# arcosoph/nanowakeword

Hardware: AMD Instinct MI355X
Metric: clips/sec (1 s @16 kHz PCM->logits) (higher is better)
Workload: dtype f32; 1 GPU; cnn head on (101,64) log-mel, batch=4096/GPU, 1 s 16 kHz mono int16 clips, 64-mel 25 ms/10 ms center frontend, fused STFT+mel HIP kernel, fp32; clips_per_gpu=4096, n_samples=16000, parallelism=batch-split x1

## Files before the change

### nanowakeword_amd/csrc/fe_steps.h

```cpp
#pragma once
#include <math.h>
#include <stdint.h>

#if defined(__HIPCC__)
#include <hip/hip_runtime.h>
#define NWW_HD __host__ __device__ __forceinline__
typedef float2 nww_c32;
#else
#define NWW_HD inline
struct nww_c32 { float x, y; };
#endif

#define FE_NFFT 400
#define FE_M 200
#define FE_BINS 201
#define FE_PSTRIDE 209
#define FE_MAX_MELS 128
#define FE_MAX_MELW 640

NWW_HD nww_c32 c_make(float x, float y) { nww_c32 r; r.x = x; r.y = y; return r; }
NWW_HD nww_c32 c_add(nww_c32 a, nww_c32 b) { return c_make(a.x + b.x, a.y + b.y); }
NWW_HD nww_c32 c_sub(nww_c32 a, nww_c32 b) { return c_make(a.x - b.x, a.y - b.y); }
NWW_HD nww_c32 c_mul(nww_c32 a, nww_c32 b) { return c_make(a.x * b.x - a.y * b.y, a.x * b.y + a.y * b.x); }
NWW_HD nww_c32 c_mul_negi(nww_c32 a) { return c_make(a.y, -a.x); }
NWW_HD nww_c32 c_scale(nww_c32 a, float s) { return c_make(a.x * s, a.y * s); }

struct FeTables {
    nww_c32 win2[FE_M];
    nww_c32 tw200[8 * 25];
    nww_c32 tw400[101];
    int32_t mel_lo[FE_MAX_MELS];
    int32_t mel_cnt[FE_MAX_MELS];
    int32_t mel_off[FE_MAX_MELS];
    float melw[FE_MAX_MELW];
};

NWW_HD void dft8(nww_c32 z[8]) {
    const float r = 0.70710678118654752440f;
    nww_c32 a0 = c_add(z[0], z[4]), a1 = c_add(z[1], z[5]), a2 = c_add(z[2], z[6]), a3 = c_add(z[3], z[7]);
    nww_c32 b0 = c_sub(z[0], z[4]);
    nww_c32 d1 = c_sub(z[1], z[5]), d2 = c_sub(z[2], z[6]), d3 = c_sub(z[3], z[7]);
    nww_c32 b1 = c_make((d1.x + d1.y) * r, (d1.y - d1.x) * r);
    nww_c32 b2 = c_mul_negi(d2);
    nww_c32 b3 = c_make((d3.y - d3.x) * r, -(d3.x + d3.y) * r);
    nww_c32 p0 = c_add(a0, a2), p1 = c_sub(a0, a2), q0 = c_add(a1, a3), q1 = c_mul_negi(c_sub(a1, a3));
    z[0] = c_add(p0, q0); z[4] = c_sub(p0, q0); z[2] = c_add(p1, q1); z[6] = c_sub(p1, q1);
    nww_c32 s0 = c_add(b0, b2), s1 = c_sub(b0, b2), t0 = c_add(b1, b3), t1 = c_mul_negi(c_sub(b1, b3));
    z[1] = c_add(s0, t0); z[5] = c_sub(s0, t0); z[3] = c_add(s1, t1); z[7] = c_sub(s1, t1);
}

NWW_HD void dft5(nww_c32& x0, nww_c32& x1, nww_c32& x2, nww_c32& x3, nww_c32& x4) {
    const float c1 = 0.30901699437494742410f, c2 = -0.80901699437494742410f;
    const float s1 = 0.95105651629515357212f, s2 = 0.58778525229247312917f;
    nww_c32 a1 = c_add(x1, x4), a2 = c_add(x2, x3), b1 = c_sub(x1, x4), b2 = c_sub(x2, x3);
    nww_c32 m1 = c_make(x0.x + c1 * a1.x + c2 * a2.x, x0.y + c1 * a1.y + c2 * a2.y);
    nww_c32 m2 = c_make(x0.x + c2 * a1.x + c1 * a2.x, x0.y + c2 * a1.y + c1 * a2.y);
    nww_c32 n1 = c_make(s1 * b1.x + s2 * b2.x, s1 * b1.y + s2 * b2.y);
    nww_c32 n2 = c_make(s2 * b1.x - s1 * b2.x, s2 * b1.y - s1 * b2.y);
    nww_c32 j1 = c_mul_negi(n1), j2 = c_mul_negi(n2);
    x0 = c_make(x0.x + a1.x + a2.x, x0.y + a1.y + a2.y);
    x1 = c_add(m1, j1); x4 = c_sub(m1, j1);
    x2 = c_add(m2, j2); x3 = c_sub(m2, j2);
}

NWW_HD nww_c32 w25(int p) {
    const float C[17] = {1.0f, 0.96858316112863108f, 0.87630668004386358f, 0.72896862742141155f,
                         0.53582679497899666f, 0.30901699437494742f, 0.06279051952931337f,
                         -0.18738131458572463f, -0.42577929156507272f, -0.63742398974868975f,
                         -0.80901699437494742f, -0.92977648588825146f, -0.99211470131447788f,
                         -0.99211470131447788f, -0.92977648588825146f, -0.80901699437494742f,
                         -0.63742398974868975f};
    const float S[17] = {0.0f, 0.24868988716485479f, 0.48175367410171532f, 0.68454710592868873f,
                         0.84432792550201508f, 0.95105651629515357f, 0.99802672842827156f,
                         0.98228725072868872f, 0.90482705246601958f, 0.77051324277578925f,
                         0.58778525229247313f, 0.36812455268467797f, 0.12533323356430426f,
                         -0.12533323356430426f, -0.36812455268467797f, -0.58778525229247313f,
                         -0.77051324277578925f};
    return c_make(C[p], -S[p]);
}

#if defined(__HIP_DEVICE_COMPILE__)
#define NWW_SCHED_FENCE() __builtin_amdgcn_sched_barrier(0)
#else
#define NWW_SCHED_FENCE() ((void)0)
#endif
template <bool SEQ = false, typename LoadF, typename StoreF>
NWW_HD void dft25(LoadF load, StoreF store) {
    nww_c32 u[5][5];
#pragma unroll
    for (int b = 0; b < 5; ++b)
#pragma unroll
        for (int a = 0; a < 5; ++a) u[b][a] = load(5 * a + b);
#pragma unroll
    for (int b = 0; b < 5; ++b) {
        if (SEQ) NWW_SCHED_FENCE();
        dft5(u[b][0], u[b][1], u[b][2], u[b][3], u[b][4]);
        if (b > 0) {
#pragma unroll
            for (int c = 1; c < 5; ++c) u[b][c] = c_mul(u[b][c], w25(b * c));
        }
    }
#pragma unroll
    for (int c = 0; c < 5; ++c) {
        if (SEQ) NWW_SCHED_FENCE();
        dft5(u[0][c], u[1][c], u[2][c], u[3][c], u[4][c]);
#pragma unroll
        for (int d = 0; d < 5; ++d) store(c + 5 * d, u[d][c]);
    }
    if (SEQ) NWW_SCHED_FENCE();
}

NWW_HD void fe_s1(int f, int n2, int hop, const int16_t* span, const FeTables* tb, nww_c32* yz) {
    const uint32_t* fr = (const uint32_t*)(span + hop * f);
    nww_c32 z[8];
#pragma unroll
    for (int n1 = 0; n1 < 8; ++n1) {
        const int m = 25 * n1 + n2;
        const nww_c32 w = tb->win2[m];
        const uint32_t v = fr[m];
        z[n1] = c_make((float)(int16_t)(v & 0xffffu) * w.x, (float)(int16_t)(v >> 16) * w.y);
    }
    dft8(z);
    nww_c32* out = yz + (f * 8) * 25 + n2;
    out[0] = z[0];
#pragma unroll
    for (int k1 = 1; k1 < 8; ++k1) out[k1 * 25] = c_mul(z[k1], tb->tw200[k1 * 25 + n2]);
}

NWW_HD void fe_s2(int f, int k1, nww_c32* yz) {
    nww_c32* row = yz + (f * 8 + k1) * 25;
    dft25([&](int i) { return row[i]; }, [&](int i, nww_c32 v) { row[i] = v; });
}

NWW_HD void fe_s3_core(nww_c32 A, nww_c32 B, nww_c32 tw, float* pa, float* pb) {
    const nww_c32 E = c_make(A.x + B.x, A.y - B.y);
    const nww_c32 O = c_make(A.y + B.y, B.x - A.x);
    const nww_c32 wO = c_mul(tw, O);
    const nww_c32 Xa = c_add(E, wO), Xb = c_sub(E, wO);
    *pa = Xa.x * Xa.x + Xa.y * Xa.y;
    *pb = Xb.x * Xb.x + Xb.y * Xb.y;
}
NWW_HD int fe_zpos(int k) { return (k & 7) * 25 + (k >> 3); }

NWW_HD void fe_s3(int f, int k, const FeTables* tb, const nww_c32* yz, float* pw) {
    const nww_c32* zf = yz + f * 200;
    const int kb = (k == 0) ? 0 : 200 - k;
    float* p = pw + f * FE_PSTRIDE;
    fe_s3_core(zf[fe_zpos(k)], zf[fe_zpos(kb)], tb->tw400[k], &p[k], &p[200 - k]);
}

NWW_HD float fe_s4(int f, int j, const FeTables* tb, const float* pw) {
    const float* p = pw + f * FE_PSTRIDE + tb->mel_lo[j];
    const float* w = tb->melw + tb->mel_off[j];
    const int n = tb->mel_cnt[j];
    float acc = 0.0f;
    for (int i = 0; i < n; ++i) acc = fmaf(p[i], w[i], acc);
    return acc;
}

NWW_HD float fe_db(float mel, float amin, float mult) {
    return mult * log10f(fmaxf(mel, amin));
}

NWW_HD int fe_reflect(int s, int N) {
    if (s < 0) s = -s;
    if (s >= N) s = 2 * (N - 1) - s;
    return s;
}

#define FE2_G 8
#define FE2_FRAME_DW 400
#define FE2_PSHIFT(f) (4 * ((f) >> 1))
#define FE2_STAGE_OFF 216
#define FE2_MAX_TILES 8
#define FE2_MAX_STEPS 512

#define FE2_CHUNK 8
#define FE2_MAX_CHUNKS 64
struct Fe2MelPlan {
    int32_t ntiles;
    int32_t total_steps;
    int32_t nchunks;
    int32_t tile_k0[FE2_MAX_TILES];
    int32_t tile_nsteps[FE2_MAX_TILES];
    int32_t tile_first[FE2_MAX_TILES];
    uint32_t chunk_meta[FE2_MAX_CHUNKS];
    float b[FE2_MAX_STEPS * 64];
};

NWW_HD void fe2_s1(const uint32_t s[8], const nww_c32 win[8], const nww_c32 tw[7], nww_c32 z[8]) {
#pragma unroll
    for (int n1 = 0; n1 < 8; ++n1)
        z[n1] = c_make((float)(int16_t)(s[n1] & 0xffffu) * win[n1].x, (float)(int16_t)(s[n1] >> 16) * win[n1].y);
    dft8(z);
#pragma unroll
    for (int k1 = 1; k1 < 8; ++k1) z[k1] = c_mul(z[k1], tw[k1 - 1]);
}

NWW_HD float fe2_mel_planned(const Fe2MelPlan* pl, const float* p, int j) {
    const int t = j >> 4, n = j & 15;
    const int k0 = pl->tile_k0[t], ns = pl->tile_nsteps[t];
    const float* b = pl->b + (size_t)pl->tile_first[t] * 64 + n;
    float acc[2] = {0.0f, 0.0f};
    for (int s = 0; s < ns; ++s)
        for (int kk = 0; kk < 4; ++kk) acc[s & 1] = fmaf(p[k0 + 4 * s + kk], b[s * 64 + kk * 16], acc[s & 1]);
    return acc[0] + acc[1];
}
```

### nanowakeword_amd/csrc/frontend2.hip

```cpp
#include <hip/hip_runtime.h>
#include <stdlib.h>
#include "fe_steps.h"
#include "frontend.h"
#include "layers.h"

typedef float f32x4 __attribute__((ext_vector_type(4)));

struct Fe2MelLds {
    uint32_t desc[FE_MAX_MELS];
    float w[FE_MAX_MELW];
};

__device__ __forceinline__ void fe2_wave_sync() {
    __builtin_amdgcn_fence(__ATOMIC_RELEASE, "wavefront");
    __builtin_amdgcn_wave_barrier();
    __builtin_amdgcn_fence(__ATOMIC_ACQUIRE, "wavefront");
}

__device__ __forceinline__ void fe2_load_column(const int16_t* __restrict__ x, int base, int n2, uint32_t v[8]) {
    const uint32_t* p = reinterpret_cast<const uint32_t*>(x + base) + n2;
#pragma unroll
    for (int n1 = 0; n1 < 8; ++n1) v[n1] = p[25 * n1];
}

__device__ __forceinline__ float fe2_db(float mel, float amin, float mult, float floor_db) {
    const float db = (mult * 0.30102999566398120f) * __log2f(fmaxf(mel, amin));
    return mel > amin ? db : floor_db;
}

#define FE2_PARAMS                                                                                                      \
    const int16_t *__restrict__ pcm, size_t row_stride, int B, int N, int T, int ngroups, int hop, int pad, int n_mels,    \
        float amin, float db_mult, float floor_db, const FeTables *__restrict__ gtb, const Fe2MelPlan *__restrict__ plan,  \
        float *__restrict__ out_db, float *__restrict__ out_mel, int frames_major, int dbg, int gsz, Fe2Sub sub
#define FE2_ARGS pcm, row_stride, B, N, T, ngroups, hop, pad, n_mels, amin, db_mult, floor_db, gtb, plan, out_db, out_mel, frames_major, dbg, gsz, sub
template <int MEL, int FAST_OUT, int MAXT, bool RING, bool FLAT>
__device__ __forceinline__ void fe2_wave_body(FE2_PARAMS) {
    static_assert(!FLAT || (FAST_OUT && !RING && MEL == 2), "flat items: frames-major fast output, register filters, no frame subsets");
#ifndef NWW_ABLATION
    if (FLAT) dbg = 0;
#endif
    extern __shared__ __attribute__((aligned(16))) char smem[];
    constexpr int MFMA_MEL = MEL == 1;
    const int lane = threadIdx.x & 63;
    const int wv = __builtin_amdgcn_readfirstlane((int)(threadIdx.x >> 6));
    const int nwv = blockDim.x >> 6;
    const int tb_bytes = MEL == 0 ? (int)sizeof(Fe2MelLds) : 0;
    Fe2MelLds* mt = reinterpret_cast<Fe2MelLds*>(smem);
    float* slab = reinterpret_cast<float*>(smem + tb_bytes) + wv * (FE2_G * FE2_FRAME_DW);
    if (MEL == 0) {
        for (int i = threadIdx.x; i < FE_MAX_MELS; i += blockDim.x)
            mt->desc[i] = (uint32_t)gtb->mel_lo[i] | ((uint32_t)gtb->mel_cnt[i] << 8) | ((uint32_t)gtb->mel_off[i] << 16);
        for (int i = threadIdx.x; i < FE_MAX_MELW; i += blockDim.x) mt->w[i] = gtb->melw[i];
        __syncthreads();
    }
    const int n2 = lane % 25, slot = lane / 25;
    nww_c32 win[8], tw[7];
#pragma unroll
    for (int n1 = 0; n1 < 8; ++n1) win[n1] = gtb->win2[25 * n1 + n2];
#pragma unroll
    for (int k1 = 1; k1 < 8; ++k1) tw[k1 - 1] = gtb->tw200[k1 * 25 + n2];
    const int k3a = lane, k3b = 64 + lane;
    const bool has_b = k3b <= 100;
    const nww_c32 twa = gtb->tw400[k3a], twb = gtb->tw400[has_b ? k3b : 100];
    const int ia2 = k3a ? FE_M - k3a : 0;
    const int f2 = lane >> 3, k1_2 = lane & 7;
    constexpr int NCO = FLAT ? 2 : 4;
    int co_off[NCO];
#pragma unroll
    for (int r = 0; r < NCO; ++r) {
        const int i = 4 * lane + 256 * r, f = i / n_mels, j = i - f * n_mels;
        co_off[r] = f * FE2_FRAME_DW + FE2_STAGE_OFF + FE2_PSHIFT(f) + j;
    }
    const int mel_l5 = lane & 31;
    const int mel_j = (lane & 32) + ((mel_l5 < 4) ? mel_l5 : (mel_l5 < 12) ? 12 + mel_l5 : (mel_l5 < 16) ? mel_l5 - 8 : (mel_l5 < 20) ? 8 + mel_l5
                                     : (mel_l5 < 28) ? mel_l5 - 12 : mel_l5);
    float wreg[MAXT];
    int mel_lo_lane = 0;
    if (MEL == 2) {
        const int j = min(mel_j, n_mels - 1);
        const int lo = gtb->mel_lo[j], sh4 = lo & 3;
        mel_lo_lane = lo - sh4;
        const int cnt = mel_j < n_mels ? gtb->mel_cnt[j] : 0, off = gtb->mel_off[j];
#pragma unroll
        for (int i = 0; i < MAXT; ++i) wreg[i] = (i >= sh4 && i - sh4 < cnt) ? gtb->melw[off + i - sh4] : 0.0f;
    }
    const int mel_nchunks = MFMA_MEL ? plan->nchunks : 0;
    const uint32_t mel_meta = MFMA_MEL ? plan->chunk_meta[lane] : 0u;
    const bool aligned = ((reinterpret_cast<uintptr_t>(pcm) | (row_stride * sizeof(int16_t))) & 3) == 0;

    const int total = FLAT ? (B * T + FE2_G - 1) / FE2_G : B * ngroups;
    const int stride = gridDim.x * nwv;
    uint32_t cur[8];
    auto geom = [&](int item, int& b, int& t0, int& nf) {
        b = item / ngroups;
        const int g = item - b * ngroups;
        if (!RING || sub.nr == 0) {
            t0 = g * gsz;
            nf = min(gsz, T - t0);
        } else {
            int r = 0;
            while (r + 1 < sub.nr && g >= sub.gend[r]) ++r;
            t0 = sub.t0[r] + (g - (r ? sub.gend[r - 1] : 0)) * gsz;
            nf = min(gsz, sub.t1[r] - t0);
        }
    };
    auto interior = [&](int t0, int nf) {
        const int s0 = t0 * hop - pad;
        return aligned && s0 >= 0 && s0 + (nf - 1) * hop + FE_NFFT <= N;
    };
    auto prefetch_first = [&](int item) {
        int b, t0, nf;
        geom(item, b, t0, nf);
        if (interior(t0, nf) && slot < nf && slot < 2)
            fe2_load_column(pcm + (size_t)b * row_stride, (t0 + slot) * hop - pad, n2, cur);
    };
    auto flat_frame = [&](int t0, int nf, int k, uint32_t& woff, int& s0) {
        int f = 2 * k + slot;
        if (nf < FE2_G) f = min(f, nf - 1);
        int t = t0 + f;
        woff = 0u;
        if (t0 + FE2_G > T)
            while (t >= T) { t -= T; woff += (uint32_t)row_stride; }
        s0 = t * hop - pad;
    };
    auto flat_load = [&](const int16_t* x, uint32_t woff, int s0, uint32_t (&v)[8]) {
        const bool edge = !aligned || __builtin_amdgcn_ballot_w64(s0 < 0 || s0 + FE_NFFT > N) != 0;
        const char* xb = reinterpret_cast<const char*>(x);
        if (!edge) {
            const uint32_t o = 2u * (woff + (uint32_t)s0 + 2u * (uint32_t)n2);
#pragma unroll
            for (int n1 = 0; n1 < 8; ++n1) v[n1] = *reinterpret_cast<const uint32_t*>(xb + o + 100 * n1);
        } else {
            uint32_t lo[8], hi[8];
#pragma unroll
            for (int n1 = 0; n1 < 8; ++n1) {
                const int q = s0 + 2 * (n2 + 25 * n1);
                lo[n1] = *reinterpret_cast<const uint16_t*>(xb + 2u * (woff + (uint32_t)fe_reflect(q, N)));
                hi[n1] = *reinterpret_cast<const uint16_t*>(xb + 2u * (woff + (uint32_t)fe_reflect(q + 1, N)));
            }
#pragma unroll
            for (int n1 = 0; n1 < 8; ++n1) v[n1] = lo[n1] | (hi[n1] << 16);
        }
    };
    auto flat_plain = [&](int t0, int nf) {
        const int s0 = t0 * hop - pad;
        return aligned && nf == FE2_G && t0 + FE2_G <= T && s0 >= 0 && s0 + (FE2_G - 1) * hop + FE_NFFT <= N;
    };
    auto plain_off = [&](int t0, int k) { return 2u * (uint32_t)((t0 + 2 * k + slot) * hop - pad + 2 * n2); };
    auto plain_load = [&](const int16_t* x, uint32_t o, uint32_t (&v)[8]) {
        const char* xb = reinterpret_cast<const char*>(x);
#pragma unroll
        for (int n1 = 0; n1 < 8; ++n1) v[n1] = *reinterpret_cast<const uint32_t*>(xb + o + 100 * n1);
    };
    auto flat_first = [&](const int16_t* x, int t0, int nf) {
        if (lane < 50) {
            if (flat_plain(t0, nf)) {
                plain_load(x, plain_off(t0, 0), cur);
            } else {
                uint32_t woff; int s0;
                flat_frame(t0, nf, 0, woff, s0);
                flat_load(x, woff, s0, cur);
            }
        }
    };
    int item = __builtin_amdgcn_readfirstlane((int)(blockIdx.x * nwv + wv));
    int fb = 0, ft = 0, fdb = 0, fdt = 0;
    if (FLAT) {
        const int g0 = FE2_G * item, step = FE2_G * stride;
        fb = g0 / T; ft = g0 - fb * T;
        fdb = step / T; fdt = step - fdb * T;
    }
    if (item < total) {
        if (FLAT) flat_first(pcm + (size_t)fb * row_stride, ft, min(FE2_G, B * T - FE2_G * item));
        else prefetch_first(item);
    }
    for (; item < total; item += stride) {
        int b, t0, nf;
        if (FLAT) { b = fb; t0 = ft; nf = min(FE2_G, B * T - FE2_G * item); }
        else geom(item, b, t0, nf);
        const int16_t* x = pcm + (size_t)b * row_stride;
        if (FLAT) {
            auto s1_trip = [&](int f) {
                if (!(dbg & 1)) {
                    nww_c32 z[8];
                    fe2_s1(cur, win, tw, z);
                    nww_c32* y = reinterpret_cast<nww_c32*>(slab + f * FE2_FRAME_DW) + n2;
#pragma unroll
                    for (int k1 = 0; k1 < 8; ++k1) y[k1 * 25] = z[k1];
                }
            };
            if (lane < 50) {
                if (flat_plain(t0, nf)) {
                    uint32_t o = plain_off(t0, 1);
#pragma unroll 1
                    for (int k = 0; k < FE2_G / 2; ++k) {
                        uint32_t nxt[8];
                        plain_load(x, o, nxt);
                        s1_trip(2 * k + slot);
#pragma unroll
                        for (int n1 = 0; n1 < 8; ++n1) cur[n1] = nxt[n1];
                        if (k + 2 < FE2_G / 2) o += 4u * (uint32_t)hop;
                    }
                } else {
#pragma unroll 1
                    for (int k = 0; k < FE2_G / 2; ++k) {
                        uint32_t nxt[8];
                        uint32_t woff; int s0;
                        flat_frame(t0, nf, min(k + 1, FE2_G / 2 - 1), woff, s0);
                        flat_load(x, woff, s0, nxt);
                        s1_trip(2 * k + slot);
#pragma unroll
                        for (int n1 = 0; n1 < 8; ++n1) cur[n1] = nxt[n1];
                    }
                }
            }
        } else {
            const bool inner = interior(t0, nf);
            const uint32_t* span = reinterpret_cast<const uint32_t*>(slab + 6 * FE2_FRAME_DW);
            if (!inner) {
                const int s0 = t0 * hop - pad, npairs = ((nf - 1) * hop + FE_NFFT) >> 1;
                uint32_t* sp = reinterpret_cast<uint32_t*>(slab + 6 * FE2_FRAME_DW);
                for (int i = lane; i < npairs; i += 64) {
                    const int q = s0 + 2 * i;
                    sp[i] = (uint32_t)(uint16_t)x[fe_reflect(q, N)] | ((uint32_t)(uint16_t)x[fe_reflect(q + 1, N)] << 16);
                }
                fe2_wave_sync();
                if (slot < nf && slot < 2) {
#pragma unroll
                    for (int n1 = 0; n1 < 8; ++n1) cur[n1] = span[((slot * hop) >> 1) + n2 + 25 * n1];
                }
            }
            const int nit = (nf + 1) >> 1;
#pragma unroll 1
            for (int it = 0; it < nit; ++it) {
                const int f = 2 * it + slot, fn = f + 2;
                uint32_t nxt[8];
#pragma unroll
                for (int n1 = 0; n1 < 8; ++n1) nxt[n1] = 0u;
                if (slot < 2 && fn < nf && it + 1 < FE2_G / 2) {
                    if (inner) {
                        fe2_load_column(x, (t0 + fn) * hop - pad, n2, nxt);
                    } else {
#pragma unroll
                        for (int n1 = 0; n1 < 8; ++n1) nxt[n1] = span[((fn * hop) >> 1) + n2 + 25 * n1];
                    }
                }
                if (slot < 2 && f < nf && !(dbg & 1)) {
                    nww_c32 z[8];
                    fe2_s1(cur, win, tw, z);
                    nww_c32* y = reinterpret_cast<nww_c32*>(slab + f * FE2_FRAME_DW) + n2;
#pragma unroll
                    for (int k1 = 0; k1 < 8; ++k1) y[k1 * 25] = z[k1];
                }
#pragma unroll
                for (int n1 = 0; n1 < 8; ++n1) cur[n1] = nxt[n1];
            }
        }
        fe2_wave_sync();
        if (f2 < nf && !(dbg & 2)) {
            nww_c32* zf = reinterpret_cast<nww_c32*>(slab + f2 * FE2_FRAME_DW);
            const nww_c32* row = zf + k1_2 * 25;
            nww_c32* dst = zf + k1_2;
            dft25<true>([&](int i) { return row[i]; }, [&](int i, nww_c32 v) { dst[8 * i] = v; });
        }
        fe2_wave_sync();
        if (FLAT) {
            fb += fdb; ft += fdt;
            if (ft >= T) { ft -= T; ++fb; }
            if (item + stride < total) flat_first(pcm + (size_t)fb * row_stride, ft, min(FE2_G, B * T - FE2_G * (item + stride)));
        } else if (item + stride < total) prefetch_first(item + stride);
        if (!(dbg & 4)) {
            const nww_c32* z0 = reinterpret_cast<const nww_c32*>(slab);
            nww_c32 a1 = z0[k3a], b1 = z0[ia2], a2 = z0[has_b ? k3b : 0], b2 = z0[has_b ? FE_M - k3b : 0];
#pragma unroll
            for (int f = 0; f < FE2_G; ++f) {
                if (f >= nf) break;
                nww_c32 na1 = a1, nb1 = b1, na2 = a2, nb2 = b2;
                if (f + 1 < FE2_G) {
                    const nww_c32* zn = reinterpret_cast<const nww_c32*>(slab + (f + 1) * FE2_FRAME_DW);
                    na1 = zn[k3a]; nb1 = zn[ia2]; na2 = zn[has_b ? k3b : 0]; nb2 = zn[has_b ? FE_M - k3b : 0];
                }
                float pa1, pb1, pa2, pb2;
                fe_s3_core(a1, b1, twa, &pa1, &pb1);
                fe_s3_core(a2, b2, twb, &pa2, &pb2);
                float* p = slab + f * FE2_FRAME_DW + FE2_PSHIFT(f);
                p[k3a] = pa1;
                p[FE_M - k3a] = pb1;
                if (has_b) { p[k3b] = pa2; p[FE_M - k3b] = pb2; }
                a1 = na1; b1 = nb1; a2 = na2; b2 = nb2;
            }
        }
        fe2_wave_sync();
        if (!(dbg & 8)) {
            if (MFMA_MEL) {
                const int fa = lane & 7;
                const float* arow = slab + fa * FE2_FRAME_DW + FE2_PSHIFT(fa) + (lane >> 4);
                const float* bp = plan->b + lane;
                f32x4 acc0 = {0.f, 0.f, 0.f, 0.f}, acc1 = {0.f, 0.f, 0.f, 0.f};
                auto load_chunk = [&](int c, float (&av)[FE2_CHUNK], float (&bv)[FE2_CHUNK]) {
                    const float* ap = arow + (__builtin_amdgcn_readlane(mel_meta, c) & 0xfff);
                    const float* bq = bp + (size_t)((dbg & 16) ? 0 : c) * (FE2_CHUNK * 64);
#pragma unroll
                    for (int s = 0; s < FE2_CHUNK; ++s) { av[s] = ap[4 * s]; bv[s] = bq[64 * s]; }
                };
                auto run_chunk = [&](int c, const float (&av)[FE2_CHUNK], const float (&bv)[FE2_CHUNK]) {
#pragma unroll
                    for (int s = 0; s < FE2_CHUNK; s += 2) {
                        acc0 = __builtin_amdgcn_mfma_f32_16x16x4f32(av[s], bv[s], acc0, 0, 0, 0);
                        acc1 = __builtin_amdgcn_mfma_f32_16x16x4f32(av[s + 1], bv[s + 1], acc1, 0, 0, 0);
                    }
                    const uint32_t meta = __builtin_amdgcn_readlane(mel_meta, c);
                    if (meta & 0x10000u) {
                        const int j = 16 * ((meta >> 12) & 0xf) + (lane & 15);
                        if (lane < 32 && j < n_mels) {
                            if (FAST_OUT) {
                                float* st = slab + (4 * (lane >> 4)) * FE2_FRAME_DW + FE2_STAGE_OFF + FE2_PSHIFT(4 * (lane >> 4)) + j;
#pragma unroll
                                for (int i = 0; i < 4; ++i)
                                    st[i * FE2_FRAME_DW + FE2_PSHIFT(i)] = fe2_db(acc0[i] + acc1[i], amin, db_mult, floor_db);
                            } else {
#pragma unroll
                                for (int i = 0; i < 4; ++i) {
                                    const int f = 4 * (lane >> 4) + i;
                                    const float m = acc0[i] + acc1[i];
                                    const float db = fe2_db(m, amin, db_mult, floor_db);
                                    if (f < nf) {
                                        if (frames_major) {
                                            slab[f * FE2_FRAME_DW + FE2_STAGE_OFF + FE2_PSHIFT(f) + j] = db;
                                            if (out_mel) out_mel[((size_t)b * T + t0 + f) * n_mels + j] = m;
                                        } else {
                                            const size_t o = ((size_t)b * n_mels + j) * T + t0 + f;
                                            if (out_db) out_db[o] = db;
                                            if (out_mel) out_mel[o] = m;
                                        }
                                    }
                                }
                            }
                        }
                        acc0 = f32x4{0.f, 0.f, 0.f, 0.f};
                        acc1 = f32x4{0.f, 0.f, 0.f, 0.f};
                    }
                };
                float a0[FE2_CHUNK], b0[FE2_CHUNK], a1[FE2_CHUNK], b1[FE2_CHUNK];
                const int last = mel_nchunks - 1;
                load_chunk(0, a0, b0);
#pragma unroll 1
                for (int c = 0; c < mel_nchunks; c += 2) {
                    load_chunk(min(c + 1, last), a1, b1);
                    run_chunk(c, a0, b0);
                    load_chunk(min(c + 2, last), a0, b0);
                    if (c + 1 < mel_nchunks) run_chunk(c + 1, a1, b1);
                }
            } else if (MEL == 2) {
                const float* p0 = slab + mel_lo_lane;
#pragma unroll 1
                for (int f = 0; f < nf; f += 2) {
                    const float* pa = p0 + f * FE2_FRAME_DW + FE2_PSHIFT(f);
                    const float* pb = pa + FE2_FRAME_DW;
                    float ma = 0.0f, mb = 0.0f;
#pragma unroll
                    for (int i = 0; i < MAXT; i += 4) {
                        const float4 a4 = *reinterpret_cast<const float4*>(__builtin_assume_aligned(pa + i, 16));
                        const float4 b4 = *reinterpret_cast<const float4*>(__builtin_assume_aligned(pb + i, 16));
                        ma = fmaf(a4.x, wreg[i], ma); mb = fmaf(b4.x, wreg[i], mb);
                        ma = fmaf(a4.y, wreg[i + 1], ma); mb = fmaf(b4.y, wreg[i + 1], mb);
                        ma = fmaf(a4.z, wreg[i + 2], ma); mb = fmaf(b4.z, wreg[i + 2], mb);
                        ma = fmaf(a4.w, wreg[i + 3], ma); mb = fmaf(b4.w, wreg[i + 3], mb);
                    }
                    if (mel_j < n_mels) {
                        const float da = fe2_db(ma, amin, db_mult, floor_db), db2 = fe2_db(mb, amin, db_mult, floor_db);
                        if (FAST_OUT) {
                            float* st = slab + f * FE2_FRAME_DW + FE2_STAGE_OFF + FE2_PSHIFT(f) + mel_j;
                            st[0] = da;
                            st[FE2_FRAME_DW] = db2;
                        } else {
#pragma unroll
                            for (int q = 0; q < 2; ++q) {
                                const int fq = f + q;
                                const float m = q ? mb : ma, db = q ? db2 : da;
                                if (fq < nf) {
                                    if (frames_major) {
                                        slab[fq * FE2_FRAME_DW + FE2_STAGE_OFF + FE2_PSHIFT(fq) + mel_j] = db;
                                        if (out_mel) out_mel[((size_t)b * T + t0 + fq) * n_mels + mel_j] = m;
                                    } else {
                                        const size_t o = ((size_t)b * n_mels + mel_j) * T + t0 + fq;
                                        if (out_db) out_db[o] = db;
                                        if (out_mel) out_mel[o] = m;
                                    }
                                }
                            }
                        }
                    }
                }
            } else {
                const int f = lane & 7;
                if (f < nf) {
                    const float* prow = slab + f * FE2_FRAME_DW + FE2_PSHIFT(f);
                    for (int j = lane >> 3; j < n_mels; j += 8) {
                        const uint32_t d = mt->desc[j];
                        const float* p = prow + (d & 0xffu);
                        const float* w = mt->w + (d >> 16);
                        const int n = (d >> 8) & 0xffu;
                        float m = 0.0f;
                        for (int i = 0; i < n; ++i) m = fmaf(p[i], w[i], m);
                        const float db = fe2_db(m, amin, db_mult, floor_db);
                        if (frames_major) {
                            slab[f * FE2_FRAME_DW + FE2_STAGE_OFF + FE2_PSHIFT(f) + j] = db;
                            if (out_mel) out_mel[((size_t)b * T + t0 + f) * n_mels + j] = m;
                        } else {
                            const size_t o = ((size_t)b * n_mels + j) * T + t0 + f;
                            if (out_db) out_db[o] = db;
                            if (out_mel) out_mel[o] = m;
                        }
                    }
                }
            }
        }
        if (frames_major && out_db) {
            fe2_wave_sync();
            const int cnt = nf * n_mels;
            if (RING && sub.ring_rows) {
                float* base = out_db + (size_t)b * sub.out_clip_stride;
                for (int i = 4 * lane; i < cnt; i += 256) {
                    const int f = i / n_mels, j = i - f * n_mels, x = sub.row0 + t0 + f;
                    const float4 v = *reinterpret_cast<const float4*>(slab + f * FE2_FRAME_DW + FE2_STAGE_OFF + FE2_PSHIFT(f) + j);
                    *reinterpret_cast<float4*>(base + (size_t)x * n_mels + j) = v;
                    *reinterpret_cast<float4*>(base + (size_t)(x < sub.ring_rows ? x + sub.ring_rows : x - sub.ring_rows) * n_mels + j) = v;
                }
            } else {
            float* dst = out_db + ((size_t)b * T + t0) * n_mels;
            if ((n_mels & 3) == 0) {
#pragma unroll
                for (int r = 0; r < NCO; ++r) {
                    const int i = 4 * lane + 256 * r;
                    if (i < cnt) *reinterpret_cast<float4*>(dst + i) = *reinterpret_cast<const float4*>(slab + co_off[r]);
                }
            } else {
                for (int i = lane; i < cnt; i += 64) {
                    const int f = i / n_mels, j = i - f * n_mels;
                    dst[i] = slab[f * FE2_FRAME_DW + FE2_STAGE_OFF + FE2_PSHIFT(f) + j];
                }
            }
            }
        }
        fe2_wave_sync();
    }
}

template <int MEL, int FAST_OUT, int MAXT, bool RING = false, bool FLAT = false>
__global__ void __launch_bounds__(256, 3) fe2_wave_kernel(FE2_PARAMS) { fe2_wave_body<MEL, FAST_OUT, MAXT, RING, FLAT>(FE2_ARGS); }

bool fe2_subset_supported(const FeParams& p, int mel_mode) { return mel_mode != 0 && (p.n_mels & 3) == 0; }

int fe2_lds_bytes(int waves, int mel_mode) {
    return waves * FE2_G * FE2_FRAME_DW * 4 + (mel_mode == 0 ? (int)sizeof(Fe2MelLds) : 0);
}

hipError_t fe2_launch(const int16_t* d_pcm, size_t row_stride, int B, int N, int T, const FeParams& p,
                      const FeTables* d_tables, const Fe2MelPlan* d_plan, float* d_db, float* d_mel, int frames_major,
                      int mel_mode, int max_taps, int block, int max_grid, hipStream_t stream, const Fe2Sub* subset) {
    if (block < 64 || block > 1024 || (block & 63)) return hipErrorInvalidValue;
    const int nwv = block / 64;
    Fe2Sub sub = subset ? *subset : Fe2Sub{};
    if (sub.nr < 0 || sub.nr > 4) return hipErrorInvalidValue;
    if ((sub.nr || sub.ring_rows) && !(frames_major && d_db && !d_mel && (p.n_mels & 3) == 0)) return hipErrorInvalidValue;
    if (sub.ring_rows && (sub.ring_rows < T || sub.row0 < 0 || sub.row0 >= sub.ring_rows)) return hipErrorInvalidValue;
    auto count_groups = [&](int g) {
        if (sub.nr == 0) return (T + g - 1) / g;
        int n = 0;
        for (int r = 0; r < sub.nr; ++r) { n += (sub.t1[r] - sub.t0[r] + g - 1) / g; sub.gend[r] = n; }
        return n;
    };
    for (int r = 0; r < sub.nr; ++r)
        if (sub.t0[r] < 0 || sub.t1[r] <= sub.t0[r] || sub.t1[r] > T) return hipErrorInvalidValue;
    int ngroups = count_groups(FE2_G);
    int mode = mel_mode;
    if (mode == 2 && (p.n_mels > 64 || max_taps > 25)) mode = 1;
    const int lds = fe2_lds_bytes(nwv, mode);
    const int fast = (frames_major && d_db && !d_mel) ? 1 : 0;
    const bool ring = sub.nr > 0 || sub.ring_rows > 0;
    if (ring && (mode == 0 || !fast)) return hipErrorInvalidValue;
#ifdef NWW_ABLATION
    static const int dbg = [] { const char* e = getenv("NWW_FE_DBG"); return e ? atoi(e) : 0; }();
#else
    const int dbg = 0;
#endif
    const int small_g = 2;
    int gsz = FE2_G;
    if (mode == 2 && small_g >= 2 && small_g < FE2_G && (small_g % 2) == 0 && (long long)B * ngroups * 4 <= (long long)max_grid * nwv) {
        gsz = small_g;
        ngroups = count_groups(gsz);
    }
    const bool flat = fast && !ring && mode == 2 && gsz == FE2_G && T != FE2_G && (long long)B * T <= 0x7fffffffLL - FE2_G &&
                      (unsigned long long)row_stride * FE2_G + (unsigned long long)N < (1ull << 31);
    auto kern = mode == 0 ? fe2_wave_kernel<0, 0, 1>
              : mode == 1 ? (ring ? fe2_wave_kernel<1, 1, 1, true> : fast ? fe2_wave_kernel<1, 1, 1> : fe2_wave_kernel<1, 0, 1>)
              : max_taps <= 17 ? (ring ? fe2_wave_kernel<2, 1, 20, true> : flat ? fe2_wave_kernel<2, 1, 20, false, true> : fast ? fe2_wave_kernel<2, 1, 20> : fe2_wave_kernel<2, 0, 20>)
                               : (ring ? fe2_wave_kernel<2, 1, 28, true> : flat ? fe2_wave_kernel<2, 1, 28, false, true> : fast ? fe2_wave_kernel<2, 1, 28> : fe2_wave_kernel<2, 0, 28>);
    const void* fn = reinterpret_cast<const void*>(kern);
    {
        hipError_t e = nww_allow_lds(fn, (size_t)lds);
        if (e != hipSuccess) return e;
    }
    const long long total = flat ? ((long long)B * T + FE2_G - 1) / FE2_G : (long long)B * ngroups;
    long long need = (total + nwv - 1) / nwv;
    int grid = (int)(need < max_grid ? need : max_grid);
    if (grid < 1) grid = 1;
    const int pad = p.center ? FE_NFFT / 2 : 0;
    hipLaunchKernelGGL(kern, dim3(grid), dim3(block), lds, stream, d_pcm, row_stride, B, N, T, ngroups, p.hop, pad, p.n_mels,
                       p.amin, p.db_mult, p.db_mult * log10f(p.amin), d_tables, d_plan, d_db, d_mel, frames_major, dbg, gsz, sub);
    return hipGetLastError();
}
```

Measured before the change: 9.365 million clips/s.

## Fuse window/twiddle into radix-8 stage, unroll flat loads, touch next PCM lines early

Merges the window multiply and the twiddle multiply into the radix-8 butterfly using explicit FMAs, with contraction turned off so the rounding pattern is fixed. The flat plain path now issues all three remaining frame loads up front instead of one per loop trip, which exposes more memory-level parallelism. It also adds a per-lane dummy load that touches the cache lines of the next work item's PCM, consumed through an empty asm, as a software prefetch. These raise register pressure and add extra global loads.

New measurement: 9.355 million clips/s, median of 2. Within noise of the previous version (-0.1%).

```diff
diff --git a/nanowakeword_amd/csrc/fe_steps.h b/nanowakeword_amd/csrc/fe_steps.h
--- a/nanowakeword_amd/csrc/fe_steps.h
+++ b/nanowakeword_amd/csrc/fe_steps.h
@@ -35,19 +35,53 @@
     float melw[FE_MAX_MELW];
 };
 
-NWW_HD void dft8(nww_c32 z[8]) {
+#if !defined(__clang__) && defined(__GNUC__)
+#pragma GCC push_options
+#pragma GCC optimize("fp-contract=off")
+#endif
+NWW_HD void fe2_s1(const uint32_t s[8], const nww_c32 win[8], const nww_c32 tw[7], nww_c32 z[8]) {
+#if defined(__clang__)
+#pragma clang fp contract(off)
+#endif
     const float r = 0.70710678118654752440f;
-    nww_c32 a0 = c_add(z[0], z[4]), a1 = c_add(z[1], z[5]), a2 = c_add(z[2], z[6]), a3 = c_add(z[3], z[7]);
-    nww_c32 b0 = c_sub(z[0], z[4]);
-    nww_c32 d1 = c_sub(z[1], z[5]), d2 = c_sub(z[2], z[6]), d3 = c_sub(z[3], z[7]);
-    nww_c32 b1 = c_make((d1.x + d1.y) * r, (d1.y - d1.x) * r);
-    nww_c32 b2 = c_mul_negi(d2);
-    nww_c32 b3 = c_make((d3.y - d3.x) * r, -(d3.x + d3.y) * r);
-    nww_c32 p0 = c_add(a0, a2), p1 = c_sub(a0, a2), q0 = c_add(a1, a3), q1 = c_mul_negi(c_sub(a1, a3));
-    z[0] = c_add(p0, q0); z[4] = c_sub(p0, q0); z[2] = c_add(p1, q1); z[6] = c_sub(p1, q1);
-    nww_c32 s0 = c_add(b0, b2), s1 = c_sub(b0, b2), t0 = c_add(b1, b3), t1 = c_mul_negi(c_sub(b1, b3));
-    z[1] = c_add(s0, t0); z[5] = c_sub(s0, t0); z[3] = c_add(s1, t1); z[7] = c_sub(s1, t1);
-}
+    float lo[8], hi[8];
+#pragma unroll
+    for (int n1 = 0; n1 < 8; ++n1) {
+        lo[n1] = (float)(int16_t)(s[n1] & 0xffffu);
+        hi[n1] = (float)(int16_t)(s[n1] >> 16);
+    }
+    nww_c32 a[4], d[4];
+#pragma unroll
+    for (int n = 0; n < 4; ++n) {
+        const float px = win[n + 4].x * lo[n + 4], py = win[n + 4].y * hi[n + 4];
+        a[n] = c_make(fmaf(win[n].x, lo[n], px), fmaf(win[n].y, hi[n], py));
+        d[n] = c_make(fmaf(win[n].x, lo[n], -px), fmaf(win[n].y, hi[n], -py));
+    }
+    const float p0x = a[0].x + a[2].x, p0y = a[0].y + a[2].y, p1x = a[0].x - a[2].x, p1y = a[0].y - a[2].y;
+    const float q0x = a[1].x + a[3].x, q0y = a[1].y + a[3].y, ex = a[1].x - a[3].x, ey = a[1].y - a[3].y;
+    z[0] = c_make(p0x + q0x, p0y + q0y);
+    const nww_c32 z4 = c_make(p0x - q0x, p0y - q0y);
+    const nww_c32 z2 = c_make(p1x + ey, p1y - ex);
+    const nww_c32 z6 = c_make(p1x - ey, p1y + ex);
+    const float sum1 = d[1].x + d[1].y, dif1 = d[1].y - d[1].x;
+    const float b3x = (d[3].y - d[3].x) * r, b3y = -((d[3].x + d[3].y) * r);
+    const float s0x = d[0].x + d[2].y, s0y = d[0].y - d[2].x, s1x = d[0].x - d[2].y, s1y = d[0].y + d[2].x;
+    const float t0x = fmaf(sum1, r, b3x), t0y = fmaf(dif1, r, b3y);
+    const float gx = fmaf(sum1, r, -b3x), gy = fmaf(dif1, r, -b3y);
+    const nww_c32 z1 = c_make(s0x + t0x, s0y + t0y), z5 = c_make(s0x - t0x, s0y - t0y);
+    const nww_c32 z3 = c_make(s1x + gy, s1y - gx), z7 = c_make(s1x - gy, s1y + gx);
+    const nww_c32 y[8] = {z[0], z1, z2, z3, z4, z5, z6, z7};
+#pragma unroll
+    for (int k1 = 1; k1 < 8; ++k1) {
+        const nww_c32 w = tw[k1 - 1], v = y[k1];
+        const float re = fmaf(v.x, w.x, -(v.y * w.y));
+        const float im = (k1 & 1) ? fmaf(v.y, w.x, v.x * w.y) : fmaf(v.x, w.y, v.y * w.x);
+        z[k1] = c_make(re, im);
+    }
+}
+#if !defined(__clang__) && defined(__GNUC__)
+#pragma GCC pop_options
+#endif
 
 NWW_HD void dft5(nww_c32& x0, nww_c32& x1, nww_c32& x2, nww_c32& x3, nww_c32& x4) {
     const float c1 = 0.30901699437494742410f, c2 = -0.80901699437494742410f;
@@ -112,19 +146,19 @@
 
 NWW_HD void fe_s1(int f, int n2, int hop, const int16_t* span, const FeTables* tb, nww_c32* yz) {
     const uint32_t* fr = (const uint32_t*)(span + hop * f);
-    nww_c32 z[8];
+    uint32_t s[8];
+    nww_c32 win[8], tw[7], z[8];
 #pragma unroll
     for (int n1 = 0; n1 < 8; ++n1) {
-        const int m = 25 * n1 + n2;
-        const nww_c32 w = tb->win2[m];
-        const uint32_t v = fr[m];
-        z[n1] = c_make((float)(int16_t)(v & 0xffffu) * w.x, (float)(int16_t)(v >> 16) * w.y);
-    }
-    dft8(z);
+        s[n1] = fr[25 * n1 + n2];
+        win[n1] = tb->win2[25 * n1 + n2];
+    }
+#pragma unroll
+    for (int k1 = 1; k1 < 8; ++k1) tw[k1 - 1] = tb->tw200[k1 * 25 + n2];
+    fe2_s1(s, win, tw, z);
     nww_c32* out = yz + (f * 8) * 25 + n2;
-    out[0] = z[0];
-#pragma unroll
-    for (int k1 = 1; k1 < 8; ++k1) out[k1 * 25] = c_mul(z[k1], tb->tw200[k1 * 25 + n2]);
+#pragma unroll
+    for (int k1 = 0; k1 < 8; ++k1) out[k1 * 25] = z[k1];
 }
 
 NWW_HD void fe_s2(int f, int k1, nww_c32* yz) {
@@ -188,15 +222,6 @@
     float b[FE2_MAX_STEPS * 64];
 };
 
-NWW_HD void fe2_s1(const uint32_t s[8], const nww_c32 win[8], const nww_c32 tw[7], nww_c32 z[8]) {
-#pragma unroll
-    for (int n1 = 0; n1 < 8; ++n1)
-        z[n1] = c_make((float)(int16_t)(s[n1] & 0xffffu) * win[n1].x, (float)(int16_t)(s[n1] >> 16) * win[n1].y);
-    dft8(z);
-#pragma unroll
-    for (int k1 = 1; k1 < 8; ++k1) z[k1] = c_mul(z[k1], tw[k1 - 1]);
-}
-
 NWW_HD float fe2_mel_planned(const Fe2MelPlan* pl, const float* p, int j) {
     const int t = j >> 4, n = j & 15;
     const int k0 = pl->tile_k0[t], ns = pl->tile_nsteps[t];
diff --git a/nanowakeword_amd/csrc/frontend2.hip b/nanowakeword_amd/csrc/frontend2.hip
--- a/nanowakeword_amd/csrc/frontend2.hip
+++ b/nanowakeword_amd/csrc/frontend2.hip
@@ -170,6 +170,12 @@
         fb = g0 / T; ft = g0 - fb * T;
         fdb = step / T; fdt = step - fdb * T;
     }
+    uint32_t touch = 0u;
+    const char* pcm_c = reinterpret_cast<const char*>(pcm);
+    const long long pcm_lo7 = (long long)(reinterpret_cast<uintptr_t>(pcm) & 127);
+    const long long t_lo = (long long)((0 - reinterpret_cast<uintptr_t>(pcm)) & 3);
+    const long long t_hi = ((pcm_lo7 + 2 * ((long long)(B - 1) * (long long)row_stride + N)) & ~3LL) - pcm_lo7 - 4;
+    const uint32_t t_lane = 128u * (uint32_t)min(lane, 23);
     if (item < total) {
         if (FLAT) flat_first(pcm + (size_t)fb * row_stride, ft, min(FE2_G, B * T - FE2_G * item));
         else prefetch_first(item);
@@ -180,10 +186,10 @@
         else geom(item, b, t0, nf);
         const int16_t* x = pcm + (size_t)b * row_stride;
         if (FLAT) {
-            auto s1_trip = [&](int f) {
+            auto s1_trip = [&](const uint32_t (&v)[8], int f) {
                 if (!(dbg & 1)) {
                     nww_c32 z[8];
-                    fe2_s1(cur, win, tw, z);
+                    fe2_s1(v, win, tw, z);
                     nww_c32* y = reinterpret_cast<nww_c32*>(slab + f * FE2_FRAME_DW) + n2;
 #pragma unroll
                     for (int k1 = 0; k1 < 8; ++k1) y[k1 * 25] = z[k1];
@@ -191,16 +197,19 @@
             };
             if (lane < 50) {
                 if (flat_plain(t0, nf)) {
-                    uint32_t o = plain_off(t0, 1);
-#pragma unroll 1
-                    for (int k = 0; k < FE2_G / 2; ++k) {
-                        uint32_t nxt[8];
-                        plain_load(x, o, nxt);
-                        s1_trip(2 * k + slot);
-#pragma unroll
-                        for (int n1 = 0; n1 < 8; ++n1) cur[n1] = nxt[n1];
-                        if (k + 2 < FE2_G / 2) o += 4u * (uint32_t)hop;
-                    }
+                    uint32_t sa[8], sb[8], sc[8];
+#ifdef NWW_ABLATION
+                    const bool abl_hot = (dbg & 32) != 0;
+#else
+                    const bool abl_hot = false;
+#endif
+                    plain_load(x, plain_off(t0, abl_hot ? 0 : 1), sa);
+                    plain_load(x, plain_off(t0, abl_hot ? 0 : 2), sb);
+                    plain_load(x, plain_off(t0, abl_hot ? 0 : 3), sc);
+                    s1_trip(cur, slot);
+                    s1_trip(sa, 2 + slot);
+                    s1_trip(sb, 4 + slot);
+                    s1_trip(sc, 6 + slot);
                 } else {
 #pragma unroll 1
                     for (int k = 0; k < FE2_G / 2; ++k) {
@@ -208,7 +217,7 @@
                         uint32_t woff; int s0;
                         flat_frame(t0, nf, min(k + 1, FE2_G / 2 - 1), woff, s0);
                         flat_load(x, woff, s0, nxt);
-                        s1_trip(2 * k + slot);
+                        s1_trip(cur, 2 * k + slot);
 #pragma unroll
                         for (int n1 = 0; n1 < 8; ++n1) cur[n1] = nxt[n1];
                     }
@@ -255,6 +264,17 @@
 #pragma unroll
                 for (int n1 = 0; n1 < 8; ++n1) cur[n1] = nxt[n1];
             }
+        }
+        if (FLAT) {
+            asm volatile("" : : "v"(touch));
+            int nb = fb + fdb, nt = ft + fdt;
+            if (nt >= T) { nt -= T; ++nb; }
+            const long long first = 2 * ((long long)nb * (long long)row_stride + (long long)(nt * hop - pad));
+            const long long line = ((first + pcm_lo7) & ~127LL) - pcm_lo7;
+            const long long rel = line < t_lo ? t_lo : line > t_hi ? t_hi : line;
+            const long long room = t_hi - rel;
+            const uint32_t room32 = room > 0x7fffffffLL ? 0x7fffffffu : (uint32_t)room;
+            touch = *reinterpret_cast<const uint32_t*>(pcm_c + rel + min(t_lane, room32 & ~3u));
         }
         fe2_wave_sync();
         if (f2 < nf && !(dbg & 2)) {
```
